# ppjian19/PhoreGen

Hardware: AMD Instinct MI355X
Metric: denoise-steps/sec (batch=128, ~40-atom graphs) (higher is better)
Workload: dtype f32; 1 GPU; BASELINE.json configs[2]: ONE batch of 128 LigPhore-shaped graphs (n~N(40,6) atoms, p~N(107,30) pharmacophore nodes), partitioned over 1 GPU(s) by the fitted step cost, steps t=999.. of the 1000-step sampler, device Philox noise, trajectory written; graphs_total=128, graphs_rank0=128, n_ctx=18401, n_lig=5115, e_knn=588832, e_bond=203720, e3=8087028, parallelism=graph-sharded x1, final RCCL gather only, triplet_workgroups_rank0=256

## Files before the change

include/phoregen_hip.h:

```cpp
#ifndef PHOREGEN_HIP_H
#define PHOREGEN_HIP_H

#include <stdint.h>

#ifdef __cplusplus
extern "C" {
#endif

const char* pg_last_error(void);
int pg_abi_version(void);
int pg_abi_struct_sizes(int* out, int n);

int pg_order_point_create(void** ev);
int pg_order_point_destroy(void* ev);
int pg_order_point_record(void* ev, void* stream);
int pg_order_point_wait(void* ev, void* stream);
int pg_debug_order_point_fence_free(int on);

enum {
  PG_OP_RECORD = 0, PG_OP_WAIT = 1, PG_OP_GEMM = 2, PG_OP_SEG_ATTN = 3, PG_OP_EMBED_CTX = 4, PG_OP_EMBED_BOND = 5, PG_OP_KNN_CTX = 6,
  PG_OP_LIG_NORMALS = 7, PG_OP_EDGE_GATE = 8, PG_OP_KNN_GROUP_BY_KIND = 9, PG_OP_BOND_SMEAR = 10, PG_OP_ATTN_FOLD_QUERY = 11,
  PG_OP_ATTN_UNFOLD_VALUE = 12, PG_OP_APPLY_DX = 13, PG_OP_LAYER_GEOM = 14, PG_OP_ROWS_LINEAR = 15, PG_OP_ATOM_COUNT = 16
};
#define PG_PROGRAM_LANES 4
#define PG_LAUNCH_MAX_ARGS 12
typedef struct {
  int32_t op;
  int32_t lane;
  int32_t ev;
  int32_t n_arg;
  uint64_t a[PG_LAUNCH_MAX_ARGS];
} PgLaunch;
int pg_program_create(const PgLaunch* list, int n, int n_events, void** prog);
int pg_program_run(void* prog, void* const* streams );
int pg_program_length(void* prog);
int pg_program_destroy(void* prog);

int pg_micro_mfma_f32(int workgroups, int iters, float* sink, double* flops, void* stream);

int pg_selftest_mfma(int* d_result, void* stream);
int pg_selftest_philox(const uint32_t* ctr_key, int n, uint32_t* out, void* stream);
int pg_debug_force_generic_seg(int mask);

typedef struct {
  const float* X;   int ldx;  int K1;
  const float* X2;  int ldx2; int K2;
  const float* W;   int ldw;
  const float* bias;
  const float* ln_gamma; const float* ln_beta;
  const float* add1; int ld_add1; const int* idx1;
  const float* add2; int ld_add2; const int* idx2;
  float out_scale;
  int   act;
  float* Y; int ldy; int M; int N;
  const int* rows;
  int add_rows;
} PgGemm;
int pg_gemm(const PgGemm* p, void* stream);
int pg_debug_gemm_streaming(int on);

typedef struct {
  int n_graphs, n_ctx, n_lig, n_phore, n_bond;
  int max_nlig;
  int max_gctx;
  const int* g_ctx_off;
  const int* g_nph;
  const int* g_nlig;
  const int* g_eid_off;
  const int* eid;
  const int* ctx_graph;
  const uint8_t* ctx_is_lig;
  const int* lig2ctx;
  const int* bond_src;
  const int* bond_dst;
  const int* bond_desc;
  const int* g_bond_off;
  const int* edge_ref;
} PgTopo;

int pg_embed_ctx(const PgTopo* t, const float* h_node_pert , const float* pos_pert ,
                 const int64_t* time_step , const float* W_node ,
                 const float* t_offset , const float* t_coeff ,
                 const float* h_phore_emb , const float* pos_phore ,
                 const int* phore2ctx , float* h_ctx , float* x_ctx ,
                 void* stream);
int pg_embed_bond(const PgTopo* t, const float* h_edge_pert , const int* bond_graph,
                  const int64_t* time_step, const float* W_edge , const float* t_offset,
                  const float* t_coeff, float* h_bond , void* stream);

// ... 175 lines not shown
```

phoregen_amd/csrc/gemm_stream.hip:

```cpp
#include <type_traits>

#include "wave_prims.h"
#include "../../include/phoregen_hip.h"

namespace pg {

typedef int i2v __attribute__((ext_vector_type(2)));

constexpr int ST_BM = 64;
constexpr int ST_STAGE = ST_BM * 128 * 4;

template <int NW , int NADD , int K1 ,
          int K2 , bool LN ,
          bool SSP = false >
__global__ __launch_bounds__(NW * 64, NW == 4 ? 2 : 1) void gemm_stream_kernel(PgGemm p, int n_tiles) {
  extern __shared__ __attribute__((aligned(1024))) char st_lds[];
  const int lane = threadIdx.x & 63;
  const int wave = __builtin_amdgcn_readfirstlane(threadIdx.x >> 6);
  const int l31 = lane & 31, kh = lane >> 5;
  const int colw = blockIdx.y * (NW * 32) + 32 * wave;
  const int col = colw + l31;

  float Wr[K1 ? 64 : 1];
  if constexpr (K1 > 0) {
    const float* wrow = p.W + (size_t)col * p.ldw + 4 * kh;
#pragma unroll
    for (int c = 0; c < 16; ++c) {
      const f4 w = *reinterpret_cast<const f4*>(wrow + 8 * c);
#pragma unroll
      for (int e = 0; e < 4; ++e) Wr[4 * c + e] = w[e];
    }
  }
  float W2r[K2 ? 10 : 1];
  if constexpr (K2 > 0) {
#pragma unroll
    for (int s2 = 0; s2 < 10; ++s2) W2r[s2] = p.W[(size_t)col * p.ldw + K1 + 10 * kh + s2];
  }
  const unsigned ldx2b = (unsigned)p.ldx2 * 4u;
  const __amdgpu_buffer_rsrc_t descX2 = __builtin_amdgcn_make_buffer_rsrc(const_cast<float*>(K2 ? p.X2 : nullptr), 0, (unsigned)p.M * ldx2b, 0x00020000);
  const unsigned voffX2 = (unsigned)l31 * ldx2b + 40u * kh;
  float xa[2][10], xb[2][10];
  auto load_x2 = [&](unsigned row0, float (&x)[2][10]) {
#pragma unroll
    for (int b = 0; b < 2; ++b) {
      const unsigned so = (row0 + 32u * b) * ldx2b;
      const i4v v0 = __builtin_amdgcn_raw_buffer_load_b128(descX2, voffX2, so, 0);
      const i4v v1 = __builtin_amdgcn_raw_buffer_load_b128(descX2, voffX2 + 16u, so, 0);
      const i2v v2 = __builtin_amdgcn_raw_buffer_load_b64(descX2, voffX2 + 32u, so, 0);
#pragma unroll
      for (int e = 0; e < 4; ++e) { x[b][e] = __builtin_bit_cast(float, (int)v0[e]); x[b][4 + e] = __builtin_bit_cast(float, (int)v1[e]); }
      x[b][8] = __builtin_bit_cast(float, (int)v2[0]);
      x[b][9] = __builtin_bit_cast(float, (int)v2[1]);
    }
  };
// ... 27 lines not shown
  f16v g1[2];
  const __amdgpu_buffer_rsrc_t descI1 = __builtin_amdgcn_make_buffer_rsrc(const_cast<int*>(NADD ? p.idx1 : nullptr), 0, (unsigned)p.M * 4u, 0x00020000);
  const __amdgpu_buffer_rsrc_t descA1 = __builtin_amdgcn_make_buffer_rsrc(const_cast<float*>(NADD ? p.add1 : nullptr), 0, 0xfffffff0u, 0x00020000);
  const unsigned ld1b = (unsigned)p.ld_add1 * 4u;
  const unsigned colb = (unsigned)col * 4u;
  const unsigned last_row0 = (unsigned)p.M - ST_BM;
  auto tile_row0 = [&](unsigned tl) { const unsigned r = tl * ST_BM; return r < last_row0 ? r : last_row0; };
  auto load_idx = [&](__amdgpu_buffer_rsrc_t dI, unsigned row0, i4v (&ix)[8]) {
#pragma unroll
    for (int e = 0; e < 8; ++e) ix[e] = __builtin_amdgcn_raw_buffer_load_b128(dI, 16u * kh, (row0 + 8u * e) * 4u, 0);
  };
  auto gather = [&](__amdgpu_buffer_rsrc_t dA, unsigned ldb, const i4v (&ix)[8], f16v (&g)[2]) {
#pragma unroll
    for (int b = 0; b < 2; ++b)
#pragma unroll
      for (int q = 0; q < 4; ++q)
#pragma unroll
        for (int t = 0; t < 4; ++t)
          g[b][4 * q + t] = __builtin_bit_cast(
              float, __builtin_amdgcn_raw_buffer_load_b32(dA, (unsigned)ix[4 * b + q][t] * ldb + colb, 0, 0));
  };

  unsigned voffA[4];
#pragma unroll
  for (int t = 0; t < 4; ++t) voffA[t] = (unsigned)(4 * kh + t) * ld1b + colb;
  auto gather_plain = [&](unsigned row0, f16v (&g)[2]) {
#pragma unroll
    for (int b = 0; b < 2; ++b)
#pragma unroll
      for (int r = 0; r < 16; ++r)
        g[b][r] = __builtin_bit_cast(float, __builtin_amdgcn_raw_buffer_load_b32(descA1, voffA[r & 3], (row0 + 32u * b + 8u * (r >> 2)) * ld1b, 0));
  };

  const unsigned tile_step = gridDim.x;
  unsigned tile = blockIdx.x;

  auto dma_tile = [&](unsigned tl, unsigned stage) {
    const unsigned row0b = tile_row0(tl) * ldxb;
    if constexpr (NW == 4) {
#pragma unroll
      for (int q = 0; q < 8; ++q) {
        const unsigned i = 2u * wave + (q >> 2), j = q & 3;
        lds_dma_1k(stage * ST_STAGE + (i * 4u + j) * 1024u, (q >> 2) ? voff_odd : voff_even, descX, row0b + i * 8u * ldxb + j * 128u);
      }
    } else {
#pragma unroll
      for (int j = 0; j < 4; ++j)
        lds_dma_1k(stage * ST_STAGE + ((unsigned)wave * 4u + j) * 1024u, voff_wave, descX, row0b + (unsigned)wave * 8u * ldxb + j * 128u);
    }
  };

  if constexpr (K2 > 0) load_x2(tile_row0(tile), xa);
  if constexpr (K1 > 0) dma_tile(tile, 0);
  if constexpr (NADD == 1) { i4v ix[8]; load_idx(descI1, tile_row0(tile), ix); gather(descA1, ld1b, ix, g1); }
  if constexpr (NADD == 2) gather_plain(tile_row0(tile), g1);

  auto body = [&](auto stage_c, auto first_c) {
    constexpr unsigned stage = decltype(stage_c)::value;
    constexpr bool first = decltype(first_c)::value;
    if constexpr (K1 > 0) {
      if constexpr (first) asm volatile("s_waitcnt vmcnt(0)\n\ts_barrier" ::: "memory");
      else asm volatile("s_waitcnt vmcnt(32)\n\ts_barrier" ::: "memory");
    }
    const unsigned next = tile + tile_step;
    float (&xc)[2][10] = stage ? xb : xa;
    float (&xn)[2][10] = stage ? xa : xb;
    i4v ix1[8];
    if constexpr (NADD == 1) load_idx(descI1, tile_row0(next), ix1);
    if constexpr (K2 > 0) load_x2(tile_row0(next), xn);
    if constexpr (K1 > 0) dma_tile(next, stage ^ 1u);

    if constexpr (LN) {
      const unsigned row = threadIdx.x >> 2, jj = threadIdx.x & 3;
      char* const base = st_lds + stage * ST_STAGE + ((row >> 3) * 4u + jj) * 1024u + (row & 7u) * 128u;
      const unsigned sw = (row >> 1) & 7u;
      f4 v[8];
#pragma unroll
      for (int q = 0; q < 8; ++q) v[q] = *reinterpret_cast<const f4*>(base + 16 * (q ^ sw));
      float sm = 0.f;
#pragma unroll
      for (int q = 0; q < 8; ++q) sm += (v[q][0] + v[q][1]) + (v[q][2] + v[q][3]);
      sm += __shfl_xor(sm, 1);
      sm += __shfl_xor(sm, 2);
      const float mu = sm * (1.f / 128.f);
      float qs = 0.f;
#pragma unroll
      for (int q = 0; q < 8; ++q)
#pragma unroll
        for (int e = 0; e < 4; ++e) { const float d = v[q][e] - mu; qs = fmaf(d, d, qs); }
      qs += __shfl_xor(qs, 1);
      qs += __shfl_xor(qs, 2);
      const float rs = 1.0f / sqrtf(qs * (1.f / 128.f) + 1e-5f);
#pragma unroll
      for (int q = 0; q < 8; ++q) {
        const unsigned k4 = 8u * jj + (unsigned)q;
        const f4 ga = lnt[k4], be = lnt[32 + k4];
        f4 o;
#pragma unroll
        for (int e = 0; e < 4; ++e) o[e] = fmaxf((v[q][e] - mu) * rs * ga[e] + be[e], 0.f);
        *reinterpret_cast<f4*>(base + 16 * (q ^ sw)) = o;
      }
      asm volatile("s_waitcnt lgkmcnt(0)\n\ts_barrier" ::: "memory");
    }
// ... 18 lines not shown
    }
    if constexpr (K1 > 0) {
      auto frag = [&](int c, int b) {
        return *reinterpret_cast<const f4*>(st_lds + rd[c & 3] + (stage * ST_STAGE + b * 16384u + (c >> 2) * 1024u));
      };
      f4 aA0 = frag(0, 0), aA1 = frag(0, 1), aB0, aB1;
#pragma unroll
      for (int c = 0; c < 16; c += 2) {
        if (c == 12) {
          if constexpr (NADD == 1) gather(descA1, ld1b, ix1, g1);
          if constexpr (NADD == 2) gather_plain(tile_row0(next), g1);
        }
        aB0 = frag(c + 1, 0); aB1 = frag(c + 1, 1);
        __builtin_amdgcn_sched_barrier(0);
#pragma unroll
        for (int e = 0; e < 4; ++e) {
          acc[0] = mfma32(aA0[e], Wr[4 * c + e], acc[0]);
          acc[1] = mfma32(aA1[e], Wr[4 * c + e], acc[1]);
        }
        if (c + 2 < 16) { aA0 = frag(c + 2, 0); aA1 = frag(c + 2, 1); }
        __builtin_amdgcn_sched_barrier(0);
#pragma unroll
        for (int e = 0; e < 4; ++e) {
          acc[0] = mfma32(aB0[e], Wr[4 * c + 4 + e], acc[0]);
          acc[1] = mfma32(aB1[e], Wr[4 * c + 4 + e], acc[1]);
        }
      }
      __builtin_amdgcn_sched_barrier(0);
    } else {
      if constexpr (NADD == 1) gather(descA1, ld1b, ix1, g1);
      if constexpr (NADD == 2) gather_plain(tile_row0(next), g1);
    }

    const unsigned row0 = tile_row0(tile);
#pragma unroll
    for (int b = 0; b < 2; ++b)
#pragma unroll
      for (int r = 0; r < 16; ++r) {
        const unsigned soff = (row0 + 32u * b + 8u * (r >> 2)) * ldyb + (unsigned)colw * 4u;
        float v = acc[b][r];
        if constexpr (LN) v *= p.out_scale;
        if constexpr (SSP) v = ssp(v);
        __builtin_amdgcn_raw_buffer_store_b32(__builtin_bit_cast(int, v), descY, voffY[r & 3], soff, 0);
      }
    tile = next;
  };

  body(std::integral_constant<unsigned, 0>{}, std::true_type{});
  while ((int)tile < n_tiles) {
    body(std::integral_constant<unsigned, 1>{}, std::false_type{});
    if ((int)tile >= n_tiles) break;
    body(std::integral_constant<unsigned, 0>{}, std::false_type{});
  }
  asm volatile("s_waitcnt vmcnt(0)" ::: "memory");
}

template <int NW, int NADD, int K1, int K2, bool LN = false, bool SSP = false>
static int launch_stream_t(const PgGemm* p, hipStream_t st) {
  const void* k = reinterpret_cast<const void*>(gemm_stream_kernel<NW, NADD, K1, K2, LN, SSP>);
  const size_t lds = K1 ? 2 * ST_STAGE + (LN ? 1024 : 0) : 0;
  if (lds) if (int rc = reserve_lds(k, lds, "pg_gemm(stream)")) return rc;
  const int n_tiles = (p->M + ST_BM - 1) / ST_BM;
  const int n_cb = p->N / (NW * 32);
  int per_cb = (NW == 4 ? 2 : 1) * kNumCU / n_cb;
  if (per_cb < 1) per_cb = 1;
  if (per_cb > n_tiles) per_cb = n_tiles;
  hipLaunchKernelGGL((gemm_stream_kernel<NW, NADD, K1, K2, LN, SSP>), dim3(per_cb, n_cb), dim3(NW * 64), lds, st, *p, n_tiles);
  return check_launch("pg_gemm(stream)");
}

bool gemm_stream_eligible(const PgGemm* p) {
  const bool k128 = p->K1 == 128 && (p->K2 == 0 || p->K2 == 20), k20 = p->K1 == 20 && p->K2 == 0;
  if (!(k128 || k20) || p->rows || (p->N & 127) || p->M < ST_BM) return false;
  if (p->act == 1) { if (p->K1 != 128 || p->K2 || p->N != 128 || p->ln_gamma || p->add1 || p->add2 || p->out_scale != 1.0f) return false; }
  else if (p->act != 0) return false;
  if (p->ln_gamma) { if (p->K1 != 128 || p->K2 || p->N != 128 || p->add1 || p->add2) return false; }
  else if (p->out_scale != 1.0f) return false;
  if ((p->ldx & 3) || ((size_t)p->X & 15) || (p->ldw & 3) || ((size_t)p->W & 15)) return false;
  if (p->K2 && ((p->ldx2 & 1) || ((size_t)p->X2 & 7))) return false;
  if (k20 && (p->ldx & 1)) return false;
  if (p->add2) return false;
  if (p->add1 && p->idx1 && (p->add_rows <= 0 || (size_t)p->add_rows * p->ld_add1 * 4 >= 0xfffff000ull)) return false;
  if (p->add1 && !p->idx1 && ((size_t)p->M * p->ld_add1 * 4 >= 0xfffff000ull || p->add1 == p->Y)) return false;
  if ((size_t)p->M * p->ldx * 4 >= 0xfffff000ull || (size_t)p->M * p->ldy * 4 >= 0xfffff000ull) return false;
  return true;
}

template <int K1, int K2>
static int launch_stream_k(const PgGemm* p, hipStream_t st) {
  const bool wide = (p->N & 255) == 0;
  const int nadd = p->add1 ? (p->idx1 ? 1 : 2) : 0;
  if (wide) {
    if (nadd == 0) return launch_stream_t<8, 0, K1, K2>(p, st);
    if (nadd == 1) return launch_stream_t<8, 1, K1, K2>(p, st);
    return launch_stream_t<8, 2, K1, K2>(p, st);
  }
  if (nadd == 0) return launch_stream_t<4, 0, K1, K2>(p, st);
  if (nadd == 1) return launch_stream_t<4, 1, K1, K2>(p, st);
  return launch_stream_t<4, 2, K1, K2>(p, st);
}

int launch_gemm_stream(const PgGemm* p, hipStream_t st) {
  if (p->ln_gamma) return launch_stream_t<4, 0, 128, 0, true>(p, st);
  if (p->act == 1) return launch_stream_t<4, 0, 128, 0, false, true>(p, st);
  if (p->K1 == 20) {
    PgGemm q = *p;
    q.X2 = p->X; q.ldx2 = p->ldx; q.K2 = 20; q.K1 = 0;
    return launch_stream_k<0, 20>(&q, st);
  }
  return p->K2 ? launch_stream_k<128, 20>(p, st) : launch_stream_k<128, 0>(p, st);
}

}
```

phoregen_amd/engine.py:

```python
import ctypes as C

import torch

from . import hip, options
from .packing import HEAD_SCALE, ModelPack


_SIDE_STREAMS = {}


_TRI_GRID_CACHE = {}


def side_streams(device_index, stream_set=0):
    key = (device_index, stream_set)
    if key not in _SIDE_STREAMS:
        with torch.cuda.device(device_index):
            _SIDE_STREAMS[key] = [torch.cuda.Stream(), torch.cuda.Stream(), torch.cuda.Stream()]
    return _SIDE_STREAMS[key]


def _f(*shape, device, zero=False):
    return (torch.zeros if zero else torch.empty)(*shape, dtype=torch.float32, device=device)

# ... 2 lines not shown
    __slots__ = ('kind', '__name__', 'ops', 'start', 'lane', 'tensors')

    def __init__(self, kind, name, ops=None, start=None, lane=0, tensors=()):
        self.kind, self.__name__, self.ops, self.start, self.lane, self.tensors = kind, name, ops, start, lane, tensors

    @property
    def name(self):
        return self.__name__


class Engine:
    def __init__(self, pack: ModelPack, plan, knn_k=32, full=True, phore_only=False):
        self.lib = hip.lib()
        self.pack, self.plan, self.k = pack, plan, knn_k
        self.dev = plan.device
        self._keep = []
        self.debug = None
        self.timers = None
        self.trace = None
        self.tri_calls = []
        o = options.snapshot()
        self.multi_stream = o['streams']
        self.layer_ahead = o['layer_ahead']
        self.tri_split, self.tri_split_from = o['tri_split'], o['tri_split_from']
        self.tri_overlap = o['tri_overlap']
        self.chain_q_from = o['chain_q_from']
        self.tune_grid = o['tune_grid']
        self.tuned_tri_grid = None
        self.geom_split = o['geom_split'] == 'always' or (o['geom_split'] == 'auto' and self.plan.n_bond < o['geom_split_below'])
        self.ahead_v2 = o['ahead_v2'] == 'always' or (o['ahead_v2'] == 'auto' and self.plan.n_bond < o['ahead_v2_below'])
        self.step_ahead = o['step_ahead']
        self.pos_tiled, self.pos_tiled_below = o['pos_tiled'], o['pos_tiled_below']
        self.tri_grid = o['tri_grid']
        self._lane = 0
        self._n_points = 0
        self._points = {}
        self.c_program = o['c_program']
        self._compiled = {}
        self._side = None
        self.stream_set = 0
        self._alloc()
        if full:
            self.prog_phore = self._build_phore_program()
            if not phore_only:
                self.prog_fwd = self._build_forward_program()
                self.prog_step = self.prog_ahead = None

    def _alloc(self):
        p, d = self.plan, self.dev
        n, E, k = p.n_ctx, p.n_bond, self.k
        w = self.ws = type('WS', (), {})()
        w.in_h_node, w.in_pos = _f(p.n_lig, 12, device=d), _f(p.n_lig, 3, device=d)
        w.in_h_edge = _f(E, 6, device=d)
        w.in_t = torch.zeros(p.n_graphs, dtype=torch.int64, device=d)
        w.in_t_next = torch.zeros(p.n_graphs, dtype=torch.int64, device=d)
        w.h_phore_ctx, w.x_phore_ctx = _f(n, 18, device=d, zero=True), _f(n, 3, device=d, zero=True)
        w.pos_phore, w.phore_norm = _f(p.n_phore, 3, device=d), _f(p.n_phore, 3, device=d)
        w.nrm_phore_ctx = _f(n, 3, device=d, zero=True)
        w.is_ex = torch.zeros(p.n_phore, dtype=torch.uint8, device=d)
        w.hp_ctx, w.Yp = _f(n, 128, device=d), _f(n, 640, device=d)
        w.enc_ctx = _f(n, 128, device=d, zero=True)
        w.hp_emb = _f(p.n_phore, 128, device=d)
        w.cnt_hid = _f(n, 256, device=d)
        w.s_all, w.s_l = _f(p.n_phore, device=d), _f(p.n_phore, device=d)
        w.count_l, w.count_u = _f(p.n_graphs, device=d), _f(p.n_graphs, device=d)
        w.h = [_f(n, 128, device=d), _f(n, 128, device=d)]
        w.h_in = _f(n, 128, device=d)
        w.x = [_f(n, 3, device=d), _f(n, 3, device=d)]
        w.hb = [_f(E, 128, device=d), _f(E, 128, device=d)]
        w.nbr = torch.zeros(n, k, dtype=torch.int32, device=d)
        w.deg = torch.zeros(n, dtype=torch.int32, device=d)
        w.ew, w.nrm, w.G = _f(n, k, device=d), _f(n, 3, device=d), _f(E, 20, device=d)
        w.Y1, w.Y2 = _f(n, 1920, device=d), _f(n, 1280, device=d)
        w.Y1b = None
        w.q = [_f(n, 128, device=d) for _ in range(4)]
        w.U, w.S = [_f(n, 2048, device=d) for _ in range(3)], [_f(n, 2048, device=d) for _ in range(3)]
        w.swn = [_f(n, 16, device=d) for _ in range(3)]
        w.aggE, w.aggB = _f(n, 128, device=d, zero=True), _f(n, 128, device=d, zero=True)
        w.lin_tmp = _f(n, 128, device=d)
        w.CsB, w.P = _f(E, 256, device=d), _f(E, 256, device=d)
        w.CsB2 = _f(E, 256, device=d)
        w.Qd = _f(E, 256, device=d)
        w.qhid, w.qT = _f(E, 128, device=d), _f(E, 128, device=d)
        w.dxe, w.dxb = _f(n, 3, device=d, zero=True), _f(n, 3, device=d, zero=True)
        w.head = _f(n, 128, device=d)
        w.head_b = _f(E, 128, device=d)
        w.out_v, w.out_bond = _f(p.n_lig, 12, device=d), _f(E, 6, device=d)

    def _call(self, prog, fn, *args):
        assert len(args) + 1 == len(fn.argtypes), (fn.__name__, len(args) + 1, len(fn.argtypes))
        prog.append((fn, args, self._lane if self.multi_stream else 0))

    def _new_point(self):
        self._n_points += 1
        return self._n_points - 1

    def _order(self, prog, name, ops):
        if self.multi_stream and ops:
            prog.append((_Tap('order', name, ops=ops), None, -1))

    def _fork(self, prog, lanes):
        if not self.multi_stream:
            return
        pt = self._new_point()
        self._order(prog, 'fork', [('record', pt, 0)] + [('wait', pt, l) for l in lanes])

    def _join(self, prog, lanes):
        self._sync(prog, 0, lanes, name='join')
# ... 19 lines not shown
            return
        self._order(prog, 'wait', [('wait', pt, waiter)])

    def _event(self, prog, name, start):
        prog.append((_Tap('event', name, start=start, lane=self._lane if self.multi_stream else 0), None, -1))

    def _mark(self, prog, name, *tensors, lane=0):
        prog.append((_Tap('mark', name, tensors=tensors, lane=lane if self.multi_stream else 0), None, -1))

    def _tap(self, tap, streams):
        if tap.kind == 'order':
            for what, pt, lane in tap.ops:
                ev = self._points.get(pt)
                if ev is None:
                    ev = self._points[pt] = hip.OrderPoint()
                if what == 'record':
                    ev.record(streams[lane])
                else:
                    ev.wait(streams[lane])
        elif tap.kind == 'event':
            if self.timers is not None:
                ev = torch.cuda.Event(enable_timing=True)
                ev.record(streams[tap.lane])
                self.timers.setdefault(tap.name, []).append((tap.start, ev))
        elif self.debug is not None:
            with torch.cuda.stream(streams[tap.lane]):
                self.debug[tap.name] = tuple(t.clone() for t in tap.tensors)

    def kernel_ms(self, name):
        evs = self.timers.get(name, [])
        return [a.elapsed_time(b) for (sa, a), (sb, b) in zip(evs[0::2], evs[1::2]) if sa and not sb]

    def _gemm(self, prog, X, K1, W, Y, M, N, bias=None, X2=None, K2=0, ln=None, add1=None, idx1=None, add2=None,
              idx2=None, scale=1.0, act=hip.ACT_NONE, rows=None):
        g = hip.PgGemm()
        g.X, g.ldx, g.K1 = X.data_ptr(), X.stride(0), K1
        g.X2, g.ldx2, g.K2 = (X2.data_ptr(), X2.stride(0), K2) if X2 is not None else (None, 0, 0)
        g.W, g.ldw = W.data_ptr(), W.stride(0)
        g.bias = hip.ptr(bias)
        g.ln_gamma, g.ln_beta = (ln[0].data_ptr(), ln[1].data_ptr()) if ln is not None else (None, None)
        g.add1, g.ld_add1, g.idx1 = (add1.data_ptr(), add1.stride(0), hip.ptr(idx1)) if add1 is not None else (None, 0, None)
        g.add2, g.ld_add2, g.idx2 = (add2.data_ptr(), add2.stride(0), hip.ptr(idx2)) if add2 is not None else (None, 0, None)
        g.out_scale, g.act = scale, act
        g.Y, g.ldy, g.M, g.N = Y.data_ptr(), Y.stride(0), M, N
        g.rows = hip.ptr(rows)
        g.add_rows = add1.size(0) if add1 is not None else 0
        self._keep += [g, X, W, Y, bias, X2, ln, add1, idx1, add2, idx2, rows]
        self._call(prog, self.lib.pg_gemm, C.byref(g))

    def _seg(self, prog, mode, n_seg, seg_ids, a, **kw):
        s = hip.PgSegAttn()
        s.mode, s.n_seg, s.seg_ids = mode, n_seg, hip.ptr(seg_ids)
        s.knn_k = self.k
        s.ln_gk, s.ln_bk, s.ln_gv, s.ln_bv = (t.data_ptr() for t in (a.ln_gk, a.ln_bk, a.ln_gv, a.ln_bv))
        for key, val in kw.items():
            setattr(s, key, val.data_ptr() if torch.is_tensor(val) else val)
            self._keep.append(val)
        self._keep += [s, seg_ids, a]
        self._call(prog, self.lib.pg_seg_attn, self.plan.topo_ref, C.byref(s))

    def _query_gemm(self, prog, a, Y, col0, h_dst_lists, buf):
        n, wq = self.plan.n_ctx, self.ws.q[buf]
        qh = Y[:, col0 + 4 * 128: col0 + 5 * 128]
        self._gemm(prog, qh, 128, a.W2q, wq, n, 128, bias=a.b2q, ln=(a.q_ln_g, a.q_ln_b), scale=HEAD_SCALE)

    def _node_attention(self, prog, mode, a, Y, col0, x, h_dst_lists, out=None, dx=None, csrc=None, buf=0, extra=None,
                        query_done=False, qbuf=None):
        w, p, n = self.ws, self.plan, self.plan.n_ctx
        wq, wU, wS, wsw = w.q[buf if qbuf is None else qbuf], w.U[buf], w.S[buf], w.swn[buf]
        blk = lambda b: Y[:, col0 + 128 * b: col0 + 128 * (b + 1)]
        if not query_done:
            self._query_gemm(prog, a, Y, col0, h_dst_lists, buf)
        knn = mode in (hip.SEG_KNN_NODE, hip.SEG_KNN_POS)
        pos = mode in (hip.SEG_KNN_POS, hip.SEG_BOND_POS)
        fused = mode != hip.SEG_PHORE
        merged = knn and len(h_dst_lists) == 2 and all(n > 0 for _, n, _ in h_dst_lists)
        lists = [h_dst_lists[0]] if merged else h_dst_lists
        for seg_ids, n_seg, is_lig in lists:
            if not fused:
                self._call(prog, self.lib.pg_attn_fold_query, wq.data_ptr(), 128, a.W2k_l.data_ptr(), n_seg,
                           seg_ids.data_ptr(), wU.data_ptr())
            kw = dict(x=x, Cdst_k=blk(0), Cdst_v=blk(1), ld_cdst=Y.stride(0), U=wU)
            if knn:
                kw.update(nrm=w.nrm, nbr=w.nbr, deg=w.deg, ew=w.ew, Csrc_k=blk(2), Csrc_v=blk(3), ld_csrc=Y.stride(0),
                          Wf_k=a.Wf_k[is_lig], Wf_v=a.Wf_v[is_lig])
                if merged:
                    ids2, n2, lig2 = h_dst_lists[1]
                    kw.update(seg_ids2=ids2, n_seg2=n2, Wf_k2=a.Wf_k[lig2], Wf_v2=a.Wf_v[lig2])
            elif mode == hip.SEG_PHORE:
                kw.update(Csrc_k=blk(2), Csrc_v=blk(3), ld_csrc=Y.stride(0), Wf_k=a.Wf_k, Wf_v=a.Wf_v)
            else:
                kw.update(Csrc_k=csrc[:, 0:128], Csrc_v=csrc[:, 128:256], ld_csrc=csrc.stride(0))
            if pos:
                kw.update(W2xv_l=a.W2xv_l, b2xv=a.b2xv, dx=dx, accumulate_dx=0)
                tiled = self.pos_tiled == 'always' or (self.pos_tiled == 'auto' and n_seg <= self.pos_tiled_below)
                if tiled:
                    kw.update(pos_tiled=1)
# ... 82 lines not shown
        lig = [(p.lig2ctx, p.n_lig, True)]
        both = [(p.lig2ctx, p.n_lig, True), (p.phore2ctx, p.n_phore, False)]
        L0 = pk.layers[0]
        self._sync(prog, 3, (2,))
        self._lane = 3
        self._embed_bond(prog, w.in_t_next)
        hb_done = self._record(prog, 3)
        self._lane = 2
        self._embed_ctx(prog, w.in_t_next, coords=False)
        self._first_layer_gemm(prog, L0, w.h_in, w.Y1)
        y1_done = self._record(prog, 2)
        self._query_gemm(prog, L0.NE, w.Y1, 0, both, 3)
        self._wait(prog, 2, hb_done)
        self._triplet_queries(prog, L0, w.hb[0], w.Y1)
        self._lane = 3
        self._wait(prog, 3, y1_done)
        self._bond_node_rows(prog, L0, w.hb[0], w.Y1)
        self._node_attention(prog, hip.SEG_BOND_NODE, L0.NB, w.Y1, 5 * 128, w.x[0], lig, out=w.aggB, csrc=w.CsB2, buf=2)
        self._lane = 0
        return prog

    def pipelined_programs(self):
        if not (self.step_ahead and self.multi_stream and self.layer_ahead and self.plan.n_tri_iters):
            return None
        if self.prog_step is None:
            tri_calls, self.tri_calls = self.tri_calls, []
            self.prog_step = self._build_forward_program(step_ahead=True)
            self.step_tri_calls, self.tri_calls = self.tri_calls, tri_calls
            self.prog_ahead = self._build_ahead_program()
        return self.prog_step, self.prog_ahead

    def _first_layer_gemm(self, prog, L, h_in, Y1):
        p, n = self.plan, self.plan.n_ctx
        self._gemm(prog, h_in, 128, L.W_node1, Y1, n, 1920, bias=L.b_node1)

    def _triplet_queries(self, prog, L, hb_in, Y1):
        w, p, E = self.ws, self.plan, self.plan.n_bond
        self._gemm(prog, hb_in, 128, L.TB.W_q_hb, w.qhid, E, 128, add1=Y1[:, 14 * 128:15 * 128], idx1=p.bond_dst)
        self._gemm(prog, w.qhid, 128, L.TB.W2q, w.qT, E, 128, bias=L.TB.b2q, ln=(L.TB.q_ln_g, L.TB.q_ln_b), scale=HEAD_SCALE)

    def _bond_node_rows(self, prog, L, hb_in, Y1):
        w, p, E = self.ws, self.plan, self.plan.n_bond
        self._gemm(prog, hb_in, 128, L.NB.W_hb, w.CsB2, E, 256, add1=Y1[:, 7 * 128:9 * 128], idx1=p.bond_src)

    def _denoiser_program(self, prog, lig, both, heads=None, pre_join=None, step_ahead=False):
        w, p, pk, lib = self.ws, self.plan, self.pack, self.lib
        n, E, t = p.n_ctx, p.n_bond, p.topo_ref
        h, x, hb = w.h, w.x, w.hb
        g = pk.gate
        self._fork(prog, (1,))
        self._lane = 1
        self._call(prog, lib.pg_knn_ctx, t, x[0].data_ptr(), self.k, w.nbr.data_ptr(), w.deg.data_ptr())
        self._call(prog, lib.pg_edge_gate, t, x[0].data_ptr(), w.nbr.data_ptr(), w.deg.data_ptr(), self.k,
                   g['W0'].data_ptr(), g['b0'].data_ptr(), g['g'].data_ptr(), g['b'].data_ptr(), g['W3'].data_ptr(),
                   C.c_float(g['b3']), w.ew.data_ptr())
        self._mark(prog, 'graph', w.nbr, w.deg, w.ew, lane=1)
        self._call(prog, lib.pg_knn_group_by_kind, t, self.k, w.nbr.data_ptr(), w.deg.data_ptr(), w.ew.data_ptr())
        self._lane = 0
        cur = 0
        staged = bool(p.n_tri_iters)
        n_layers = len(pk.layers)
        ahead = self.layer_ahead and self.multi_stream
        v2 = self.ahead_v2 and ahead
        chain_q = self.multi_stream and (v2 or E >= self.chain_q_from)
        tri_grid = self.tri_grid if self.tri_grid >= 0 else ((192 if E < 15000 else 224 if E < 80000 else 0) if self.multi_stream else 0)
        self._tune = None
        if (self.tune_grid and self.tri_grid < 0 and self.multi_stream and staged and 0 < tri_grid <= 224):
# ... 84 lines not shown
            self._event(prog, 'triplet', False)
            if last:
                self._fork(prog, (3,))
                self._lane = 3
                heads[0](hbn)
            self._lane = 3 if v2 else 2
            if not pre:
                bond_node_rows(L, hbc, Y1c)
                self._node_attention(prog, hip.SEG_BOND_NODE, L.NB, Y1c, 5 * 128, xc, lig, out=w.aggB, csrc=w.CsB2, buf=1)
                if v2:
                    bn_done = self._record(prog, 3)
            self._lane = 1
            if not pre:
                self._query_gemm(prog, L.NE, Y1c, 0, both, 0)
            if pre0:
                self._sync(prog, 1, (2,))
            elif pre and v2:
                self._wait(prog, 1, ne_done)
            self._event(prog, 'knn_node', True)
            self._node_attention(prog, hip.SEG_KNN_NODE, L.NE, Y1c, 0, xc1, both, out=w.aggE, buf=0, query_done=True,
                                 qbuf=3 if pre else None)
            self._event(prog, 'knn_node', False)
            if pre0:
                self._sync(prog, 1, (3,))
            elif pre or v2:
                self._wait(prog, 1, bn_done)
            else:
                self._sync(prog, 1, (2,))
            self._gemm(prog, w.aggE, 128, L.W_lin2[:, :128], w.lin_tmp, n, 128, bias=L.b_lin, add1=hc)
            self._gemm(prog, w.aggB, 128, L.W_lin2[:, 128:], hn, n, 128, add1=w.lin_tmp)
            self._mark(prog, f'A{li}', w.aggE, w.aggB, lane=1)
            if early:
                hn_done = self._record(prog, 1)
            self._gemm(prog, hn, 128, L.W_node2, w.Y2, n, 1280, bias=L.b_node2)
            if v2:
                self._query_gemm(prog, L.PB, w.Y2, 5 * 128, lig, 1)
            more_ahead = ahead and li + 1 < n_layers and not last
            self._sync(prog, 0, (1,))
            if v2 and more_ahead:
                self._lane = 1
                first_layer_gemm(pk.layers[li + 1], hn, Y1n)
                y1_done = self._record(prog, 1)
            qlane = 2 if last else 3
            if early:
                self._wait(prog, 2, hn_done)
                self._lane = 2
                heads[1](hn)
                if not v2:
                    self._fork(prog, (2,))
            else:
                self._fork(prog, (2, 3) if (ahead and li + 1 < n_layers) else (qlane,))
            self._lane = qlane
            if not v2:
                self._query_gemm(prog, L.PB, w.Y2, 5 * 128, lig, 1)
                q_done = self._record(prog, qlane)
            if last and not early:
                heads[1](hn)
            elif ahead and li + 1 < n_layers:
                Ln = pk.layers[li + 1]
                self._lane = 2
                if v2:
                    self._wait(prog, 2, y1_done)
                else:
                    first_layer_gemm(Ln, hn, Y1n)
                    y1_done = self._record(prog, 2)
                triplet_queries(Ln, hbn, Y1n)
                if not v2:
# ... 270 lines not shown
```

phoregen_amd/hip.py:

```python
import ctypes as C
import struct
import sys
import os

import torch

_HERE = os.path.dirname(os.path.abspath(__file__))
LIB_PATH = os.path.join(_HERE, '_lib', 'libphoregen_hip.so')

c_fp = C.c_void_p
c_ip = C.c_void_p


class PgGemm(C.Structure):
    _fields_ = [('X', c_fp), ('ldx', C.c_int), ('K1', C.c_int),
                ('X2', c_fp), ('ldx2', C.c_int), ('K2', C.c_int),
                ('W', c_fp), ('ldw', C.c_int),
                ('bias', c_fp),
                ('ln_gamma', c_fp), ('ln_beta', c_fp),
                ('add1', c_fp), ('ld_add1', C.c_int), ('idx1', c_ip),
                ('add2', c_fp), ('ld_add2', C.c_int), ('idx2', c_ip),
                ('out_scale', C.c_float), ('act', C.c_int),
                ('Y', c_fp), ('ldy', C.c_int), ('M', C.c_int), ('N', C.c_int), ('rows', c_ip), ('add_rows', C.c_int)]


class PgTopo(C.Structure):
    _fields_ = [('n_graphs', C.c_int), ('n_ctx', C.c_int), ('n_lig', C.c_int), ('n_phore', C.c_int),
                ('n_bond', C.c_int), ('max_nlig', C.c_int), ('max_gctx', C.c_int),
                ('g_ctx_off', c_ip), ('g_nph', c_ip), ('g_nlig', c_ip), ('g_eid_off', c_ip), ('eid', c_ip),
                ('ctx_graph', c_ip), ('ctx_is_lig', c_ip), ('lig2ctx', c_ip), ('bond_src', c_ip),
                ('bond_dst', c_ip), ('bond_desc', c_ip), ('g_bond_off', c_ip), ('edge_ref', c_ip)]


class PgSegAttn(C.Structure):
    _fields_ = [('mode', C.c_int), ('n_seg', C.c_int), ('seg_ids', c_ip), ('seg_chunks', c_ip),
                ('x', c_fp), ('nrm', c_fp), ('nbr', c_ip), ('deg', c_ip), ('ew', c_fp), ('knn_k', C.c_int),
                ('Csrc_k', c_fp), ('Csrc_v', c_fp), ('ld_csrc', C.c_int),
                ('Cdst_k', c_fp), ('Cdst_v', c_fp), ('ld_cdst', C.c_int),
                ('Wf_k', c_fp), ('Wf_v', c_fp), ('Wg2_k', c_fp), ('Wg2_v', c_fp), ('G', c_fp),
                ('ln_gk', c_fp), ('ln_bk', c_fp), ('ln_gv', c_fp), ('ln_bv', c_fp),
                ('U', c_fp), ('q', c_fp), ('W2k_l', c_fp), ('W2v_l', c_fp), ('b2v', c_fp),
                ('W2xv_l', c_fp), ('b2xv', c_fp),
                ('S', c_fp), ('swn', c_fp), ('resid', c_fp), ('out', c_fp), ('dx', c_fp),
                ('accumulate_dx', C.c_int), ('alpha', c_fp), ('alpha_rows', C.c_int), ('efeat', c_fp), ('efeat_off', c_ip),
                ('tri_iters', c_ip), ('n_tri_iters', C.c_int), ('tri_counter', c_ip),
                ('seg_ids2', c_ip), ('n_seg2', C.c_int), ('Wf_k2', c_fp), ('Wf_v2', c_fp), ('tri_grid', C.c_int), ('pos_tiled', C.c_int), ('tri_max_nlig', C.c_int)]


class PgSegAttnGrad(C.Structure):
    _fields_ = [('gS', c_fp), ('gswn', c_fp), ('gdx', c_fp), ('gU', c_fp),
                ('gCdst_k', c_fp), ('gCdst_v', c_fp), ('ld_gcdst', C.c_int),
                ('gCsrc_k', c_fp), ('gCsrc_v', c_fp), ('ld_gcsrc', C.c_int),
                ('gWf_k', c_fp), ('gWf_v', c_fp), ('gbk', c_fp), ('gbv', c_fp),
                ('gW2xv_l', c_fp), ('gb2xv', c_fp), ('gx', c_fp), ('gnrm', c_fp), ('gew', c_fp),
                ('alpha', c_fp), ('alpha_rows', C.c_int), ('S', c_fp), ('swn', c_fp),
                ('rowbuf', c_fp), ('rowbuf_rows', C.c_int), ('grid', C.c_int), ('atom_order', c_ip),
# ... 218 lines not shown
```

phoregen_amd/options.py:

```python
import contextlib
import os

DEFAULTS = dict(
    streams=True,
    layer_ahead=True,
    ahead_v2='auto',
    ahead_v2_below=82000,
    pos_tiled='auto',
    pos_tiled_below=1500,
    step_ahead=True,
    c_program=True,
    geom_split='auto',
    geom_split_below=16000,
    tune_grid=True,
    chain_q_from=150000,
    tri_split=True,
    tri_split_from=82000,
    tri_overlap=3,
    tri_grid=-1,
    dgrad_mm=True,
    rows_sum=True,
    tri_onepass=True,
    wide_gemm=True,
    bwd_atom_sort=True,
    bwd_split='all',
    bwd_grid=256,
    tri_bwd_form=2,
    tri_bwd_grid=256,
    ph_onepass=True,
)

_tri = lambda v: {'0': 'never', '1': 'auto', '2': 'always'}[v]
_flag = lambda v: v != '0'
_ENV = {
    'PG_STREAMS': ('streams', _flag),
    'PG_LAYER_AHEAD': ('layer_ahead', _flag), 'PG_AHEAD_V2': ('ahead_v2', _tri), 'PG_AHEAD_V2_BELOW': ('ahead_v2_below', int), 'PG_TRI_GRID': ('tri_grid', int), 'PG_POS_TILED': ('pos_tiled', _tri), 'PG_POS_TILED_BELOW': ('pos_tiled_below', int), 'PG_C_PROGRAM': ('c_program', _flag), 'PG_STEP_AHEAD': ('step_ahead', _flag), 'PG_CHAIN_Q_FROM': ('chain_q_from', int), 'PG_TRI_SPLIT': ('tri_split', _flag), 'PG_TUNE_GRID': ('tune_grid', _flag), 'PG_GEOM_SPLIT': ('geom_split', _tri),
    'PG_DGRAD_MM': ('dgrad_mm', _flag),
    'PG_ROWS_SUM': ('rows_sum', _flag), 'PG_TRI_ONEPASS': ('tri_onepass', _flag), 'PG_WIDE_GEMM': ('wide_gemm', _flag), 'PG_BWD_GRID': ('bwd_grid', int), 'PG_BWD_SPLIT': ('bwd_split', lambda v: {'0': 'none', '1': 'knn', '2': 'all'}[v]), 'PG_BWD_ATOM_SORT': ('bwd_atom_sort', _flag),
    'PG_TRI_BWD_FORM': ('tri_bwd_form', int), 'PG_TRI_BWD_GRID': ('tri_bwd_grid', int), 'PG_PH_ONEPASS': ('ph_onepass', _flag),
}
_overrides = {}


def get(name):
    if name in _overrides:
        return _overrides[name]
    if os.environ.get('PHOREGEN_DEBUG') == '1':
        for var, (key, conv) in _ENV.items():
            if key == name and var in os.environ:
                return conv(os.environ[var])
    return DEFAULTS[name]


def snapshot():
    return {k: get(k) for k in DEFAULTS}


@contextlib.contextmanager
def override(**kw):
    unknown = set(kw) - set(DEFAULTS)
    if unknown:
        raise KeyError(f'phoregen_amd.options: unknown switch(es) {sorted(unknown)}')
    old = dict(_overrides)
    _overrides.update(kw)
    try:
        yield
    finally:
        _overrides.clear()
        _overrides.update(old)
# ... 1 lines not shown
```

phoregen_amd/plan.py:

```python
import ctypes as C

import torch

from . import hip


class BatchPlan:
    def __init__(self, batch_node, batch_phore, edge_index, batch_edge, n_graphs, device):
        bn, bp = batch_node.detach().cpu().long(), batch_phore.detach().cpu().long()
        ei, be = edge_index.detach().cpu().long(), batch_edge.detach().cpu().long()
        B = int(n_graphs)
        if bn.numel() and (bn[1:] < bn[:-1]).any() or bp.numel() and (bp[1:] < bp[:-1]).any():
            raise ValueError('phoregen_amd: batch vectors must be sorted by graph id')
        nlig = torch.bincount(bn, minlength=B)
        nph = torch.bincount(bp, minlength=B)
        self.n_graphs, self.n_lig, self.n_phore, self.n_bond = B, int(bn.numel()), int(bp.numel()), int(ei.size(1))
        self.n_ctx = self.n_lig + self.n_phore
        if int((nlig * (nlig - 1)).sum()) != self.n_bond:
            raise ValueError('phoregen_amd: the bond graph must be the fully connected directed ligand graph '
                             '(utils/sample_utils.py:40-54 / datasets/transform.py:488-501)')
        tot = nlig + nph
        g_ctx_off = torch.zeros(B + 1, dtype=torch.long)
        g_ctx_off[1:] = tot.cumsum(0)
        lig_off = torch.zeros(B + 1, dtype=torch.long)
# ... 12 lines not shown
        g_eid_off = torch.zeros(B + 1, dtype=torch.long)
        g_eid_off[1:] = (nlig * nlig).cumsum(0)
        ls, ld = ei[0] - lig_off[be], ei[1] - lig_off[be]
        if self.n_bond and ((ls < 0).any() or (ld < 0).any() or (ls >= nlig[be]).any() or (ld >= nlig[be]).any()
                            or (bn[ei[0]] != be).any()):
            raise ValueError('phoregen_amd: edge_index / batch_edge inconsistent with batch_node')
        if self.n_bond and (be[1:] < be[:-1]).any():
            raise ValueError('phoregen_amd: bond edges must be grouped by graph (batch_edge ascending)')
        nmax = int(nlig.max()) + 1 if B else 1
        order = torch.argsort((be * nmax + ld) * nmax + ls, stable=True) if self.n_bond else torch.zeros(0, dtype=torch.long)
        self.edge_identity = bool(torch.equal(order, torch.arange(self.n_bond)))
        ei_ref, ei = ei, ei[:, order]
        ls, ld = ls[order], ld[order]
        inv = torch.empty_like(order)
        inv[order] = torch.arange(self.n_bond)
        eid = torch.full((int(g_eid_off[-1]),), -1, dtype=torch.long)
        eid[g_eid_off[be] + ls * nlig[be] + ld] = torch.arange(self.n_bond)
        if int((eid >= 0).sum()) != self.n_bond:
            raise ValueError('phoregen_amd: duplicate bond edges')

        self.device = device
        i32 = lambda t: t.to(torch.int32).to(device)
        self.num_atoms = nlig
        self.g_ctx_off, self.g_nph, self.g_nlig, self.g_eid_off = i32(g_ctx_off), i32(nph), i32(nlig), i32(g_eid_off)
        self.eid, self.ctx_graph, self.ctx_is_lig = i32(eid), i32(ctx_graph), is_lig.to(device)
        self.lig2ctx, self.phore2ctx = i32(lig2ctx), i32(phore2ctx)
        self.lig2ctx_long = lig2ctx.to(device)
        self.phore2ctx_long = phore2ctx.to(device)
        self.bond_src, self.bond_dst = i32(lig2ctx[ei[0]]), i32(lig2ctx[ei[1]])
        self.bond_graph, self.lig_graph, self.phore_graph = i32(be), i32(bn), i32(bp)
        self.bond_desc = i32(torch.stack([lig2ctx[ei[0]], ld + (ls << 16), nlig[be], g_eid_off[be]], 1).contiguous()) \
            if self.n_bond else torch.zeros(0, 4, dtype=torch.int32, device=device)
        self.g_lig_off = i32(lig_off)
        bond_off = torch.zeros(B + 1, dtype=torch.long)
        bond_off[1:] = torch.bincount(be, minlength=B).cumsum(0)
        self.g_bond_off = i32(bond_off)
        self.batch_node, self.batch_edge, self.edge_index = bn.to(device), be.to(device), ei_ref.to(device)
        self.edge_ref, self.edge_int = i32(order), i32(inv)
        self.edge_ref_long, self.edge_int_long = order.to(device), inv.to(device)

        t = hip.PgTopo()
        t.n_graphs, t.n_ctx, t.n_lig, t.n_phore, t.n_bond = B, self.n_ctx, self.n_lig, self.n_phore, self.n_bond
        t.max_nlig = int(nlig.max()) if B else 0
        t.max_gctx = int(tot.max()) if B else 0
        order = torch.argsort(ei[0], stable=True) if self.n_bond else torch.zeros(0, dtype=torch.long)
        self.tri_order = i32(order)
        cost = ((nlig[be[order]] + 15) // 16).double() + 1.0
        csum = torch.cat([torch.zeros(1, dtype=torch.double), cost.cumsum(0)])
        targets = torch.linspace(0, float(csum[-1]), 257, dtype=torch.double)
        self.tri_chunks = i32(torch.searchsorted(csum, targets).clamp(max=self.n_bond))
        self.tri_chunks[0], self.tri_chunks[-1] = 0, self.n_bond
        rows_cap, waves = 80, 12
        groups = []
        for gi in range(B):
            n = int(nlig[gi])
            if n < 2 or n - 1 > rows_cap or n > 96:
                continue
            A = max(1, min(rows_cap // (n - 1), n))
            for j0 in range(0, n, A):
                groups.append((gi, n, j0, min(A, n - j0)))
        want_parts = 1 if len(groups) >= 2 * 256 or not groups else 2

        def queue(grps):
            its = []
            for gi, n, j0, a in grps:
                tiles = (n - 2 + 15) // 16
# ... 109 lines not shown
```

Measured before the change: 54.51 steps/s.

## Compute ligand-only GEMM column blocks over ligand row tiles only

Adds a row-tile form of the streaming GEMM, where column blocks whose outputs are consumed only by ligand rows iterate over a precomputed table of contiguous ligand row ranges instead of all context rows. The node GEMMs and the ligand-only query GEMM pass a column mask marking those blocks. Stores are bounded per tile through buffer descriptors, and output buffers are zero-initialised so that the pharmacophore rows it no longer writes hold defined values. This cuts the MFMA and memory work for pharmacophore rows (about 72% of context rows), at the cost of partial tiles at graph boundaries and a more involved grid split.

```diff
diff --git a/include/phoregen_hip.h b/include/phoregen_hip.h
--- a/include/phoregen_hip.h
+++ b/include/phoregen_hip.h
@@ -55,6 +55,7 @@
   float* Y; int ldy; int M; int N;
   const int* rows;
   int add_rows;
+  const int* row_tiles; int n_row_tiles; uint32_t row_tile_cols;
 } PgGemm;
 int pg_gemm(const PgGemm* p, void* stream);
 int pg_debug_gemm_streaming(int on);
diff --git a/phoregen_amd/csrc/gemm_stream.hip b/phoregen_amd/csrc/gemm_stream.hip
--- a/phoregen_amd/csrc/gemm_stream.hip
+++ b/phoregen_amd/csrc/gemm_stream.hip
@@ -12,14 +12,37 @@
 
 template <int NW , int NADD , int K1 ,
           int K2 , bool LN ,
-          bool SSP = false >
+          bool SSP = false ,
+          bool RT = false >
 __global__ __launch_bounds__(NW * 64, NW == 4 ? 2 : 1) void gemm_stream_kernel(PgGemm p, int n_tiles) {
+  static_assert(!RT || (NADD == 0 && K1 == 128 && K2 == 0 && !SSP), "row-tile form: plain K = 128 products");
   extern __shared__ __attribute__((aligned(1024))) char st_lds[];
   const int lane = threadIdx.x & 63;
   const int wave = __builtin_amdgcn_readfirstlane(threadIdx.x >> 6);
   const int l31 = lane & 31, kh = lane >> 5;
   const int colw = blockIdx.y * (NW * 32) + 32 * wave;
   const int col = colw + l31;
+
+  typedef const __attribute__((address_space(4))) int* tile_tab_t;
+  tile_tab_t tt = nullptr;
+  unsigned tile_step = gridDim.x;
+  unsigned r0_cur = 0, nr_cur = 0, r0_nxt = 0, nr_nxt = 0;
+  if constexpr (RT) {
+    const bool sub = (p.row_tile_cols >> (blockIdx.y * (NW / 4))) & 1u;
+    tile_step = sub ? ((unsigned)n_tiles >> 16) : ((unsigned)n_tiles & 0xffffu);
+    if (blockIdx.x >= tile_step) return;
+    n_tiles = sub ? p.n_row_tiles : (p.M + ST_BM - 1) / ST_BM;
+    if (sub) tt = (tile_tab_t)(p.row_tiles);
+  }
+  auto tile_info = [&](unsigned tl, unsigned& r0, unsigned& nr) {
+    if (tl >= (unsigned)n_tiles) tl = (unsigned)n_tiles - 1u;
+    int a = (int)(tl * ST_BM), b = ST_BM;
+    if (tt) { a = tt[2 * tl]; b = tt[2 * tl + 1]; }
+    if (b > ST_BM) b = ST_BM;
+    if (b > p.M - a) b = p.M - a;
+    if (a < 0 || b <= 0) { a = 0; b = 0; }
+    r0 = (unsigned)a; nr = (unsigned)b;
+  };
 
   float Wr[K1 ? 64 : 1];
   if constexpr (K1 > 0) {
@@ -113,11 +136,10 @@
         g[b][r] = __builtin_bit_cast(float, __builtin_amdgcn_raw_buffer_load_b32(descA1, voffA[r & 3], (row0 + 32u * b + 8u * (r >> 2)) * ld1b, 0));
   };
 
-  const unsigned tile_step = gridDim.x;
   unsigned tile = blockIdx.x;
 
-  auto dma_tile = [&](unsigned tl, unsigned stage) {
-    const unsigned row0b = tile_row0(tl) * ldxb;
+  auto dma_tile = [&](unsigned row0, unsigned stage) {
+    const unsigned row0b = row0 * ldxb;
     if constexpr (NW == 4) {
 #pragma unroll
       for (int q = 0; q < 8; ++q) {
@@ -132,7 +154,8 @@
   };
 
   if constexpr (K2 > 0) load_x2(tile_row0(tile), xa);
-  if constexpr (K1 > 0) dma_tile(tile, 0);
+  if constexpr (RT) { tile_info(tile, r0_cur, nr_cur); tile_info(tile + tile_step, r0_nxt, nr_nxt); }
+  if constexpr (K1 > 0) dma_tile(RT ? r0_cur : tile_row0(tile), 0);
   if constexpr (NADD == 1) { i4v ix[8]; load_idx(descI1, tile_row0(tile), ix); gather(descA1, ld1b, ix, g1); }
   if constexpr (NADD == 2) gather_plain(tile_row0(tile), g1);
 
@@ -149,7 +172,9 @@
     i4v ix1[8];
     if constexpr (NADD == 1) load_idx(descI1, tile_row0(next), ix1);
     if constexpr (K2 > 0) load_x2(tile_row0(next), xn);
-    if constexpr (K1 > 0) dma_tile(next, stage ^ 1u);
+    unsigned r0_nn = 0, nr_nn = 0;
+    if constexpr (RT) tile_info(next + tile_step, r0_nn, nr_nn);
+    if constexpr (K1 > 0) dma_tile(RT ? r0_nxt : tile_row0(next), stage ^ 1u);
 
     if constexpr (LN) {
       const unsigned row = threadIdx.x >> 2, jj = threadIdx.x & 3;
@@ -234,17 +259,36 @@
       if constexpr (NADD == 2) gather_plain(tile_row0(next), g1);
     }
 
-    const unsigned row0 = tile_row0(tile);
-#pragma unroll
-    for (int b = 0; b < 2; ++b)
-#pragma unroll
-      for (int r = 0; r < 16; ++r) {
-        const unsigned soff = (row0 + 32u * b + 8u * (r >> 2)) * ldyb + (unsigned)colw * 4u;
-        float v = acc[b][r];
-        if constexpr (LN) v *= p.out_scale;
-        if constexpr (SSP) v = ssp(v);
-        __builtin_amdgcn_raw_buffer_store_b32(__builtin_bit_cast(int, v), descY, voffY[r & 3], soff, 0);
-      }
+    if constexpr (RT) {
+#pragma unroll
+      for (int b = 0; b < 2; ++b)
+#pragma unroll
+        for (int q = 0; q < 4; ++q) {
+          const int left = (int)nr_cur - (32 * b + 8 * q);
+          const unsigned bytes = left > 0 ? (unsigned)left * ldyb : 0u;
+          const __amdgpu_buffer_rsrc_t dY = __builtin_amdgcn_make_buffer_rsrc(
+              reinterpret_cast<char*>(p.Y) + (size_t)((r0_cur + 32u * b + 8u * q) * ldyb), 0, bytes, 0x00020000);
+#pragma unroll
+          for (int t = 0; t < 4; ++t) {
+            float v = acc[b][4 * q + t];
+            if constexpr (LN) v *= p.out_scale;
+            __builtin_amdgcn_raw_buffer_store_b32(__builtin_bit_cast(int, v), dY, voffY[t], (unsigned)colw * 4u, 0);
+          }
+        }
+      r0_cur = r0_nxt; nr_cur = nr_nxt; r0_nxt = r0_nn; nr_nxt = nr_nn;
+    } else {
+      const unsigned row0 = tile_row0(tile);
+#pragma unroll
+      for (int b = 0; b < 2; ++b)
+#pragma unroll
+        for (int r = 0; r < 16; ++r) {
+          const unsigned soff = (row0 + 32u * b + 8u * (r >> 2)) * ldyb + (unsigned)colw * 4u;
+          float v = acc[b][r];
+          if constexpr (LN) v *= p.out_scale;
+          if constexpr (SSP) v = ssp(v);
+          __builtin_amdgcn_raw_buffer_store_b32(__builtin_bit_cast(int, v), descY, voffY[r & 3], soff, 0);
+        }
+    }
     tile = next;
   };
 
@@ -268,6 +312,33 @@
   if (per_cb < 1) per_cb = 1;
   if (per_cb > n_tiles) per_cb = n_tiles;
   hipLaunchKernelGGL((gemm_stream_kernel<NW, NADD, K1, K2, LN, SSP>), dim3(per_cb, n_cb), dim3(NW * 64), lds, st, *p, n_tiles);
+  return check_launch("pg_gemm(stream)");
+}
+
+static bool rows_form(const PgGemm* p) {
+  if (!p->row_tiles || p->n_row_tiles <= 0 || !p->row_tile_cols) return false;
+  if (p->K1 != 128 || p->K2 || p->add1 || p->add2 || p->act != 0 || p->N > 32 * 128) return false;
+  return (p->N == 32 * 128) || !(p->row_tile_cols >> (p->N / 128));
+}
+
+template <int NW, bool LN>
+static int launch_stream_rows(const PgGemm* p, hipStream_t st) {
+  const void* k = reinterpret_cast<const void*>(gemm_stream_kernel<NW, 0, 128, 0, LN, false, true>);
+  const size_t lds = 2 * ST_STAGE + (LN ? 1024 : 0);
+  if (int rc = reserve_lds(k, lds, "pg_gemm(stream)")) return rc;
+  const int n_cb = p->N / (NW * 32);
+  int cb_sub = 0;
+  for (int c = 0; c < n_cb; ++c) cb_sub += (p->row_tile_cols >> (c * (NW / 4))) & 1u;
+  const int cb_all = n_cb - cb_sub;
+  const int t_all = (p->M + ST_BM - 1) / ST_BM, t_sub = p->n_row_tiles;
+  const int slots = (NW == 4 ? 2 : 1) * kNumCU;
+  int r = 1;
+  auto need = [&](int r_) { return cb_all * ((t_all + r_ - 1) / r_) + cb_sub * ((t_sub + r_ - 1) / r_); };
+  while (need(r) > slots && r < (t_all > t_sub ? t_all : t_sub)) ++r;
+  const int per_all = cb_all ? (t_all + r - 1) / r : 0, per_sub = cb_sub ? (t_sub + r - 1) / r : 0;
+  if (per_all > 0xffff || per_sub > 0xffff) { set_error("pg_gemm(stream): too many column blocks for the row-tile form"); return PG_ERR_ARG; }
+  hipLaunchKernelGGL((gemm_stream_kernel<NW, 0, 128, 0, LN, false, true>), dim3(per_all > per_sub ? per_all : per_sub, n_cb), dim3(NW * 64),
+                     lds, st, *p, per_all | (per_sub << 16));
   return check_launch("pg_gemm(stream)");
 }
 
@@ -303,6 +374,12 @@
 }
 
 int launch_gemm_stream(const PgGemm* p, hipStream_t st) {
+  if (rows_form(p)) {
+    if (p->ln_gamma) return launch_stream_rows<4, true>(p, st);
+    const unsigned m = p->row_tile_cols;
+    const bool wide = (p->N & 255) == 0 && !(((m >> 1) ^ m) & 0x55555555u);
+    return wide ? launch_stream_rows<8, false>(p, st) : launch_stream_rows<4, false>(p, st);
+  }
   if (p->ln_gamma) return launch_stream_t<4, 0, 128, 0, true>(p, st);
   if (p->act == 1) return launch_stream_t<4, 0, 128, 0, false, true>(p, st);
   if (p->K1 == 20) {
diff --git a/phoregen_amd/engine.py b/phoregen_amd/engine.py
--- a/phoregen_amd/engine.py
+++ b/phoregen_amd/engine.py
@@ -58,6 +58,7 @@
         self.step_ahead = o['step_ahead']
         self.pos_tiled, self.pos_tiled_below = o['pos_tiled'], o['pos_tiled_below']
         self.tri_grid = o['tri_grid']
+        self.gemm_rows = o['gemm_rows'] and plan.n_lig_row_tiles > 0
         self._lane = 0
         self._n_points = 0
         self._points = {}
@@ -97,9 +98,9 @@
         w.nbr = torch.zeros(n, k, dtype=torch.int32, device=d)
         w.deg = torch.zeros(n, dtype=torch.int32, device=d)
         w.ew, w.nrm, w.G = _f(n, k, device=d), _f(n, 3, device=d), _f(E, 20, device=d)
-        w.Y1, w.Y2 = _f(n, 1920, device=d), _f(n, 1280, device=d)
+        w.Y1, w.Y2 = _f(n, 1920, device=d, zero=True), _f(n, 1280, device=d, zero=True)
         w.Y1b = None
-        w.q = [_f(n, 128, device=d) for _ in range(4)]
+        w.q = [_f(n, 128, device=d, zero=True) for _ in range(4)]
         w.U, w.S = [_f(n, 2048, device=d) for _ in range(3)], [_f(n, 2048, device=d) for _ in range(3)]
         w.swn = [_f(n, 16, device=d) for _ in range(3)]
         w.aggE, w.aggB = _f(n, 128, device=d, zero=True), _f(n, 128, device=d, zero=True)
@@ -185,7 +186,7 @@
         return [a.elapsed_time(b) for (sa, a), (sb, b) in zip(evs[0::2], evs[1::2]) if sa and not sb]
 
     def _gemm(self, prog, X, K1, W, Y, M, N, bias=None, X2=None, K2=0, ln=None, add1=None, idx1=None, add2=None,
-              idx2=None, scale=1.0, act=hip.ACT_NONE, rows=None):
+              idx2=None, scale=1.0, act=hip.ACT_NONE, rows=None, lig_cols=0):
         g = hip.PgGemm()
         g.X, g.ldx, g.K1 = X.data_ptr(), X.stride(0), K1
         g.X2, g.ldx2, g.K2 = (X2.data_ptr(), X2.stride(0), K2) if X2 is not None else (None, 0, 0)
@@ -197,6 +198,8 @@
         g.out_scale, g.act = scale, act
         g.Y, g.ldy, g.M, g.N = Y.data_ptr(), Y.stride(0), M, N
         g.rows = hip.ptr(rows)
+        if lig_cols and self.gemm_rows:
+            g.row_tiles, g.n_row_tiles, g.row_tile_cols = self.plan.lig_row_tiles.data_ptr(), self.plan.n_lig_row_tiles, lig_cols
         g.add_rows = add1.size(0) if add1 is not None else 0
         self._keep += [g, X, W, Y, bias, X2, ln, add1, idx1, add2, idx2, rows]
         self._call(prog, self.lib.pg_gemm, C.byref(g))
@@ -215,7 +218,8 @@
     def _query_gemm(self, prog, a, Y, col0, h_dst_lists, buf):
         n, wq = self.plan.n_ctx, self.ws.q[buf]
         qh = Y[:, col0 + 4 * 128: col0 + 5 * 128]
-        self._gemm(prog, qh, 128, a.W2q, wq, n, 128, bias=a.b2q, ln=(a.q_ln_g, a.q_ln_b), scale=HEAD_SCALE)
+        lig_only = all(is_lig for _, _, is_lig in h_dst_lists)
+        self._gemm(prog, qh, 128, a.W2q, wq, n, 128, bias=a.b2q, ln=(a.q_ln_g, a.q_ln_b), scale=HEAD_SCALE, lig_cols=1 if lig_only else 0)
 
     def _node_attention(self, prog, mode, a, Y, col0, x, h_dst_lists, out=None, dx=None, csrc=None, buf=0, extra=None,
                         query_done=False, qbuf=None):
@@ -364,7 +368,7 @@
 
     def _first_layer_gemm(self, prog, L, h_in, Y1):
         p, n = self.plan, self.plan.n_ctx
-        self._gemm(prog, h_in, 128, L.W_node1, Y1, n, 1920, bias=L.b_node1)
+        self._gemm(prog, h_in, 128, L.W_node1, Y1, n, 1920, bias=L.b_node1, lig_cols=0x7fe0)
 
     def _triplet_queries(self, prog, L, hb_in, Y1):
         w, p, E = self.ws, self.plan, self.plan.n_bond
@@ -515,7 +519,7 @@
             self._mark(prog, f'A{li}', w.aggE, w.aggB, lane=1)
             if early:
                 hn_done = self._record(prog, 1)
-            self._gemm(prog, hn, 128, L.W_node2, w.Y2, n, 1280, bias=L.b_node2)
+            self._gemm(prog, hn, 128, L.W_node2, w.Y2, n, 1280, bias=L.b_node2, lig_cols=0x3f3)
             if v2:
                 self._query_gemm(prog, L.PB, w.Y2, 5 * 128, lig, 1)
             more_ahead = ahead and li + 1 < n_layers and not last
diff --git a/phoregen_amd/hip.py b/phoregen_amd/hip.py
--- a/phoregen_amd/hip.py
+++ b/phoregen_amd/hip.py
@@ -21,7 +21,8 @@
                 ('add1', c_fp), ('ld_add1', C.c_int), ('idx1', c_ip),
                 ('add2', c_fp), ('ld_add2', C.c_int), ('idx2', c_ip),
                 ('out_scale', C.c_float), ('act', C.c_int),
-                ('Y', c_fp), ('ldy', C.c_int), ('M', C.c_int), ('N', C.c_int), ('rows', c_ip), ('add_rows', C.c_int)]
+                ('Y', c_fp), ('ldy', C.c_int), ('M', C.c_int), ('N', C.c_int), ('rows', c_ip), ('add_rows', C.c_int),
+                ('row_tiles', c_ip), ('n_row_tiles', C.c_int), ('row_tile_cols', C.c_uint32)]
 
 
 class PgTopo(C.Structure):
diff --git a/phoregen_amd/options.py b/phoregen_amd/options.py
--- a/phoregen_amd/options.py
+++ b/phoregen_amd/options.py
@@ -17,6 +17,7 @@
     tri_split=True,
     tri_split_from=82000,
     tri_overlap=3,
+    gemm_rows=True,
     tri_grid=-1,
     dgrad_mm=True,
     rows_sum=True,
@@ -34,7 +35,7 @@
 _flag = lambda v: v != '0'
 _ENV = {
     'PG_STREAMS': ('streams', _flag),
-    'PG_LAYER_AHEAD': ('layer_ahead', _flag), 'PG_AHEAD_V2': ('ahead_v2', _tri), 'PG_AHEAD_V2_BELOW': ('ahead_v2_below', int), 'PG_TRI_GRID': ('tri_grid', int), 'PG_POS_TILED': ('pos_tiled', _tri), 'PG_POS_TILED_BELOW': ('pos_tiled_below', int), 'PG_C_PROGRAM': ('c_program', _flag), 'PG_STEP_AHEAD': ('step_ahead', _flag), 'PG_CHAIN_Q_FROM': ('chain_q_from', int), 'PG_TRI_SPLIT': ('tri_split', _flag), 'PG_TUNE_GRID': ('tune_grid', _flag), 'PG_GEOM_SPLIT': ('geom_split', _tri),
+    'PG_LAYER_AHEAD': ('layer_ahead', _flag), 'PG_AHEAD_V2': ('ahead_v2', _tri), 'PG_AHEAD_V2_BELOW': ('ahead_v2_below', int), 'PG_TRI_GRID': ('tri_grid', int), 'PG_POS_TILED': ('pos_tiled', _tri), 'PG_POS_TILED_BELOW': ('pos_tiled_below', int), 'PG_C_PROGRAM': ('c_program', _flag), 'PG_STEP_AHEAD': ('step_ahead', _flag), 'PG_CHAIN_Q_FROM': ('chain_q_from', int), 'PG_TRI_SPLIT': ('tri_split', _flag), 'PG_TUNE_GRID': ('tune_grid', _flag), 'PG_GEOM_SPLIT': ('geom_split', _tri), 'PG_GEMM_ROWS': ('gemm_rows', _flag),
     'PG_DGRAD_MM': ('dgrad_mm', _flag),
     'PG_ROWS_SUM': ('rows_sum', _flag), 'PG_TRI_ONEPASS': ('tri_onepass', _flag), 'PG_WIDE_GEMM': ('wide_gemm', _flag), 'PG_BWD_GRID': ('bwd_grid', int), 'PG_BWD_SPLIT': ('bwd_split', lambda v: {'0': 'none', '1': 'knn', '2': 'all'}[v]), 'PG_BWD_ATOM_SORT': ('bwd_atom_sort', _flag),
     'PG_TRI_BWD_FORM': ('tri_bwd_form', int), 'PG_TRI_BWD_GRID': ('tri_bwd_grid', int), 'PG_PH_ONEPASS': ('ph_onepass', _flag),
diff --git a/phoregen_amd/plan.py b/phoregen_amd/plan.py
--- a/phoregen_amd/plan.py
+++ b/phoregen_amd/plan.py
@@ -68,6 +68,16 @@
         self.bond_desc = i32(torch.stack([lig2ctx[ei[0]], ld + (ls << 16), nlig[be], g_eid_off[be]], 1).contiguous()) \
             if self.n_bond else torch.zeros(0, 4, dtype=torch.int32, device=device)
         self.g_lig_off = i32(lig_off)
+        tiles, r0, r1 = [], 0, 0
+        for gi in range(B + 1):
+            a = int(g_ctx_off[gi] + nph[gi]) if gi < B else -1
+            if a != r1:
+                tiles += [(s, min(64, r1 - s)) for s in range(r0, r1, 64)]
+                r0 = r1 = a
+            if gi < B:
+                r1 = a + int(nlig[gi])
+        self.lig_row_tiles = torch.tensor(tiles, dtype=torch.int32).reshape(-1, 2).to(device)
+        self.n_lig_row_tiles = len(tiles)
         bond_off = torch.zeros(B + 1, dtype=torch.long)
         bond_off[1:] = torch.bincount(be, minlength=B).cumsum(0)
         self.g_bond_off = i32(bond_off)
```

New measurement: 54.56 steps/s, median of 6. About the same (+0.1%).
